# klae01/ddim-audio

Measured on AMD Instinct MI355X. Metric: DDIM denoising steps/sec (U-Net fwd/s), 1000-step sample, spectrogram batch, higher is better.
Workload: dtype bf16; 1 GPU; BASELINE configs[1]: batch 8/GPU x [2,1024,256] spectrograms, audio.yml U-Net (47.2M params, hash-filled weights; FNet GEMM operands bf16), generalized_steps eta=0 over the 1000-step schedule, one hipGraph per step (inside the forward two batch shards on two streams, fork mask 0x1003f); global_batch=8, t_size=1024, parallelism=batch-sharded x1, no collective in the loop

## Files before the change

ddim_audio_amd/_lib.py:

```python
import ctypes
import os
import re
from ctypes import Structure, c_char_p, c_double, c_float, c_int, c_longlong, c_uint, c_ulonglong, c_void_p

_HERE = os.path.dirname(os.path.abspath(__file__))
LIB_PATH = os.environ.get("DDIMX_LIB", os.path.join(_HERE, "libddimx.so"))
_HEADER = os.path.join(os.path.dirname(_HERE), "include", "ddimx.h")
_DISTILL_HEADER = os.path.join(os.path.dirname(_HERE), "include", "ddimx_distill.h")
_THRESHOLD_HEADER = os.path.join(os.path.dirname(_HERE), "include", "ddimx_threshold.h")
_SDE_HEADER = os.path.join(os.path.dirname(_HERE), "include", "ddimx_sde.h")
_BROWNIAN_HEADER = os.path.join(os.path.dirname(_HERE), "include", "ddimx_brownian.h")
_WINDOW_HEADER = os.path.join(os.path.dirname(_HERE), "include", "ddimx_window.h")
_WINDOW_INPAINT_HEADER = os.path.join(os.path.dirname(_HERE), "include", "ddimx_window_inpaint.h")
_UNIC_HEADER = os.path.join(os.path.dirname(_HERE), "include", "ddimx_unic.h")

_SCALARS = {"int": c_int, "unsigned": c_uint, "long long": c_longlong, "unsigned long long": c_ulonglong, "float": c_float,
            "double": c_double}
_RETURNS = {"int": c_int, "long long": c_longlong, "const char*": c_char_p}


def parse_header(text):
    def bad(what, decl):
        return RuntimeError(f"ddimx.h: {what}: `{decl}`")

    def split(decl):
        m = re.fullmatch(r"(.*?)\b(\w+)(?:\[(\w+)\])?", decl)
        if not m or not m.group(1):
            raise bad("cannot parse", decl)
        ctype, dim = m.group(1).strip(), m.group(3)
# ... 51 lines not shown
SDE_EXPORTS = tuple(_SDE_FUNCS)
with open(_BROWNIAN_HEADER) as _f:
    _BROWNIAN_CONSTS, _, _BROWNIAN_FUNCS = parse_header(_f.read())
globals().update(_BROWNIAN_CONSTS)
BROWNIAN_EXPORTS = tuple(_BROWNIAN_FUNCS)
with open(_WINDOW_HEADER) as _f:
    _, _, _WINDOW_FUNCS = parse_header(_f.read())
WINDOW_EXPORTS = tuple(_WINDOW_FUNCS)
with open(_WINDOW_INPAINT_HEADER) as _f:
    _, _, _WINDOW_INPAINT_FUNCS = parse_header(_f.read())
WINDOW_INPAINT_EXPORTS = tuple(_WINDOW_INPAINT_FUNCS)
with open(_UNIC_HEADER) as _f:
    _UNIC_CONSTS, _, _UNIC_FUNCS = parse_header(_f.read())
globals().update(_UNIC_CONSTS)
UNIC_EXPORTS = tuple(_UNIC_FUNCS)


class DdimxConfig(Structure):
    _fields_ = _STRUCTS["ddimx_config"]


class DdimxTables(Structure):
    _fields_ = _STRUCTS["ddimx_tables"]

    def __init__(self, posenc=None, dft_hidden=None, dft_seq=None, temb_table=None):
        super().__init__(posenc, dft_hidden, dft_seq, temb_table)


_lib = None


def load():
    global _lib
    if _lib is None:
        if not os.path.exists(LIB_PATH):
            raise RuntimeError(
                f"{LIB_PATH} not found: build it with `python -m ddim_audio_amd.build` "
                "(hipcc, gfx950). The HIP library is the only compute path of ddim_audio_amd.")
        lib = ctypes.CDLL(LIB_PATH)
        for name, (res, args) in (list(_FUNCS.items()) + list(_DISTILL_FUNCS.items()) + list(_THRESHOLD_FUNCS.items()) + list(_SDE_FUNCS.items())
                                  + list(_BROWNIAN_FUNCS.items()) + list(_WINDOW_FUNCS.items()) + list(_WINDOW_INPAINT_FUNCS.items())
                                  + list(_UNIC_FUNCS.items())):
            fn = getattr(lib, name)
            fn.restype, fn.argtypes = res, args
        if lib.ddimx_abi_version() != _CONSTS["DDIMX_ABI_VERSION"]:
            raise RuntimeError("libddimx ABI version mismatch")
        _lib = lib
    return _lib


def check(rc):
    if rc != 0:
        raise RuntimeError("libddimx: " + load().ddimx_last_error().decode(errors="replace"))


def ptr(t):
    return None if t is None else c_void_p(t.data_ptr())
# ... 6 lines not shown
```

ddim_audio_amd/build.py:

```python
import os
import subprocess
import sys
from concurrent.futures import ThreadPoolExecutor

HERE = os.path.dirname(os.path.abspath(__file__))
CSRC = os.path.join(HERE, "csrc")
OUT = os.path.join(HERE, "libddimx.so")
SOURCES = ["plan.cpp", "conv_dispatch.cpp", "blocks.cpp", "walk_infer.cpp", "walk_train.cpp", "ops.cpp", "samplers.cpp", "distill.cpp", "threshold.cpp", "sde.cpp", "brownian.cpp", "window_solver.cpp", "window_inpaint.cpp", "unic.cpp",
           "edge_conv.hip", "gn_kernels.hip", "fnet_pointwise.hip", "temb_kernels.hip", "step_kernels.hip", "tail_kernels.hip",
           "pack_kernels.hip", "wgrad_reduce.hip", "gemm.hip", "fnet_dense.hip", "conv_inst_bf16_c3.hip", "conv_inst_bf16_du.hip",
           "conv_inst_f32_c3.hip", "conv_inst_f32_du.hip", "conv_inst_bf16_c3b.hip", "conv_inst_bf16_wreg.hip", "conv_inst_bf16_pipe.hip", "conv_inst_f32_c3b.hip", "wgrad_inst_bf16.hip", "wgrad_inst_f32.hip",
           "inpaint_kernels.hip", "solver_kernels.hip", "noise_kernels.hip", "window_kernels.hip", "invert_kernels.hip", "pool_kernels.hip",
           "vpred_kernels.hip", "distill_kernels.hip", "threshold_kernels.hip", "sde_kernels.hip", "brownian_kernels.hip", "window_solver_kernels.hip", "window_inpaint_kernels.hip", "unic_kernels.hip"]
FLAGS = ["--offload-arch=gfx950", "-O3", "-std=c++17", "-fPIC", "-x", "hip", "-Wno-unused-result"]
EXTRA_FLAGS = {"conv_inst_bf16_pipe.hip": ["-fno-slp-vectorize", "-mllvm", "-amdgpu-mfma-vgpr-form=1"]}


def _stale(target, deps):
    if not os.path.exists(target):
        return True
    t = os.path.getmtime(target)
    return any(os.path.getmtime(d) > t for d in deps)


def build(force=False, verbose=True, jobs=None, stamp=False):
    global OUT, FLAGS
    hipcc = os.environ.get("HIPCC", "/opt/rocm/bin/hipcc")
    bdir = os.path.join(CSRC, "build_stamp" if stamp else "build")
    if stamp:
        OUT = os.path.join(HERE, "libddimx_stamp.so")
        FLAGS = FLAGS + ["-DDDIMX_STAMP"]
    os.makedirs(bdir, exist_ok=True)
    headers = [os.path.join(CSRC, f) for f in os.listdir(CSRC) if f.endswith(".h")]
    headers += [os.path.join(os.path.dirname(HERE), "include", h) for h in ("ddimx.h", "ddimx_distill.h", "ddimx_threshold.h", "ddimx_sde.h", "ddimx_brownian.h", "ddimx_window.h", "ddimx_window_inpaint.h", "ddimx_unic.h")]
    todo, objs = [], []
    for src in SOURCES:
        sp = os.path.join(CSRC, src)
        ob = os.path.join(bdir, src.rsplit(".", 1)[0] + ".o")
        objs.append(ob)
        if force or _stale(ob, [sp] + headers):
            todo.append((sp, ob))

    def cc(job):
        sp, ob = job
        cmd = [hipcc] + FLAGS + EXTRA_FLAGS.get(os.path.basename(sp), []) + ["-c", sp, "-o", ob]
        r = subprocess.run(cmd, capture_output=True, text=True)
        if r.returncode != 0:
            raise RuntimeError("hipcc failed for %s:\n%s" % (sp, r.stderr[-4000:]))
        return sp
# ... 19 lines not shown
```

ddim_audio_amd/csrc/edge_conv.h:

```cpp
#pragma once
#include "common.h"

namespace ddimx {

enum { EDGE_CONV_IN = 0, EDGE_CONV_OUT = 1, EDGE_CONV_OUT_BWD_DATA = 2, EDGE_CONV_IN_BWD_DATA = 3, EDGE_WGRAD = 4 };
struct EdgePlan {
    int variant;
    unsigned grid_x, grid_y;
    int threads, lds;
    int trips;
    int tiles_x, tiles_y;
    int partial_blocks;
    int reduce_blocks, reduce_unrolled, reduce_tail;
};
const char* edge_plan(int op, int dtype, int B, int C0, int Cio, int H, int W, int groups, EdgePlan* p);

hipError_t conv_in_launch(int dtype, const float* x, const float* w , const float* bias, void* out,
                          float* stats, int B, int cin, int C0, int H, int W, hipStream_t s, int groups = 0);
int conv_in_nparts(int H, int W);
hipError_t conv_out_launch(int dtype, const void* a, const void* b, const float* w ,
                           const float* bias, float* out, int B, int C0, int cout, int H, int W, hipStream_t s);

hipError_t conv_out_bwd_data_launch(int dtype, const float* d_eps, const float* w , void* ds, int B, int C0,
                                    int cout, int H, int W, hipStream_t s);
hipError_t conv_in_bwd_data_launch(int dtype, const void* dy, const float* w, float* dx, int B, int C0, int NI, int H, int W,
                                   hipStream_t s);
size_t edge_wgrad_partial_floats(int dtype, int B, int C, int NI, int H, int W);
hipError_t edge_wgrad_launch(int dtype, int mode, const void* g1, const void* g2, const float* S, float* partial, float* dW,
                             float* db, int B, int C, int NI, int H, int W, hipStream_t s);

}
```

ddim_audio_amd/csrc/edge_conv.hip:

```cpp
#include "edge_conv.h"
#include "gn_fused.h"
#include <stdarg.h>
#include <stdio.h>
#include <string.h>

namespace ddimx {

constexpr int kInPixPerBlock = 1024;
constexpr int kTileH = 8, kTileW = 32;
constexpr int kEdgeT = 16;
constexpr int kEdgeChunk = 32;
constexpr int kStripRows = 128;
static inline int edge_pixb(int dtype) { return dtype == DT_BF16 ? 64 : 32; }
int conv_in_nparts(int H, int W) { return (int)(((long long)H * W + kInPixPerBlock - 1) / kInPixPerBlock); }

template <typename T>
__global__ void __launch_bounds__(256) conv_in_kernel(const float* __restrict__ x, const float* __restrict__ w,
                                                      const float* __restrict__ bias, T* __restrict__ out,
                                                      float* __restrict__ stats, int cin, int C0, int H, int W,
                                                      int groups) {
    constexpr int EPB = Piece<T>::N;
    extern __shared__ __attribute__((aligned(16))) float lds[];
    float* wl = lds;
    float* red = lds + cin * 9 * C0;
// ... 216 lines not shown
        for (int k = 0; k < 9; ++k) {
            const float v = tile[((py + k / 3) * IW + px + k % 3) * LS + ci];
#pragma unroll
            for (int o = 0; o < 4; ++o)
                if (o < cout) acc[o] = fmaf(v, w[((size_t)k * cout + o) * C0 + ci], acc[o]);
        }
    }
    const int gy = y0 + py, gx = x0 + px;
    if (gy < H && gx < W) {
#pragma unroll
        for (int o = 0; o < 4; ++o)
            if (o < cout) out[(((size_t)b * cout + o) * H + gy) * W + gx] = acc[o];
    }
}

template <typename T, int C0, int NO, bool TWO, bool BIAS>
__device__ __forceinline__ void edge_tile_conv(const T* __restrict__ a, const T* __restrict__ b2, const float* __restrict__ w,
                                               const float* __restrict__ bias, float* __restrict__ out, int H, int W, int tiles_x,
                                               int tiles_y) {
    constexpr int EPB = Piece<T>::N, ES = sizeof(T);
    constexpr int IH = kTileH + 2, IW = kTileW + 2;
    constexpr int CPP = C0 / EPB, PS = C0 * ES + 16;
    __shared__ __attribute__((aligned(16))) char tile[IH * IW * PS];
    const int tid = threadIdx.x;
    const int tx = blockIdx.x % tiles_x, ty = (blockIdx.x / tiles_x) % tiles_y, b = blockIdx.x / (tiles_x * tiles_y);
    const int y0 = ty * kTileH, x0 = tx * kTileW;
    constexpr int NPIECE = IH * IW * CPP, NIT = (NPIECE + 255) / 256;
    uint4 va[NIT], vb[TWO ? NIT : 1];
    bool inb[NIT];
#pragma unroll
    for (int u = 0; u < NIT; ++u) {
        const int i0 = tid + u * 256, i = i0 < NPIECE ? i0 : NPIECE - 1;
        const int c = i % CPP, pix = i / CPP;
        const int gy = y0 - 1 + pix / IW, gx = x0 - 1 + pix % IW;
// ... 9 lines not shown
        uint4 v;
        if constexpr (TWO) {
            float f[EPB], k[EPB];
            Piece<T>::unpack(va[u], f);
            Piece<T>::unpack(vb[u], k);
#pragma unroll
            for (int j = 0; j < EPB; ++j) f[j] += k[j];
            v = Piece<T>::pack(f);
            if (!inb[u]) v = make_uint4(0, 0, 0, 0);
        } else {
            v = inb[u] ? va[u] : make_uint4(0, 0, 0, 0);
        }
        if (i < NPIECE) *(uint4*)(tile + (i / CPP) * PS + (i % CPP) * 16) = v;
    }
    __syncthreads();
    const int py = tid / kTileW, px = tid % kTileW;
    float acc[NO];
#pragma unroll
    for (int o = 0; o < NO; ++o) acc[o] = BIAS ? bias[o] : 0.f;
#pragma unroll 1
    for (int k = 0; k < 9; ++k) {
        const char* tp = tile + ((py + k / 3) * IW + px + k % 3) * PS;
        const float* wk = w + k * NO * C0;
#pragma unroll
        for (int c = 0; c < CPP; ++c) {
            float f[EPB];
            Piece<T>::unpack(*(const uint4*)(tp + c * 16), f);
#pragma unroll
            for (int j = 0; j < EPB; ++j)
#pragma unroll
                for (int o = 0; o < NO; ++o) acc[o] = fmaf(f[j], wk[o * C0 + c * EPB + j], acc[o]);
        }
    }
    const int gy = y0 + py, gx = x0 + px;
    if (gy < H && gx < W) {
#pragma unroll
        for (int o = 0; o < NO; ++o) out[(((size_t)b * NO + o) * H + gy) * W + gx] = acc[o];
    }
}

template <typename T, int C0, int COUT>
__global__ void __launch_bounds__(256) conv_out_fast_kernel(const T* __restrict__ a, const T* __restrict__ b2,
                                                            const float* __restrict__ w, const float* __restrict__ bias,
                                                            float* __restrict__ out, int H, int W, int tiles_x,
                                                            int tiles_y) {
    edge_tile_conv<T, C0, COUT, true, true>(a, b2, w, bias, out, H, W, tiles_x, tiles_y);
}

hipError_t conv_out_launch(int dtype, const void* a, const void* b, const float* w, const float* bias, float* out, int B,
                           int C0, int cout, int H, int W, hipStream_t s) {
    EdgePlan p;
    if (edge_plan(EDGE_CONV_OUT, dtype, B, C0, cout, H, W, 0, &p)) return hipErrorInvalidValue;
    const dim3 grid(p.grid_x);
    const int tiles_x = p.tiles_x, tiles_y = p.tiles_y;
    dispatch_dtype(dtype, [&](auto t) {
        using T = typename decltype(t)::type;
        if (p.variant)
            hipLaunchKernelGGL((conv_out_fast_kernel<T, 32, 2>), grid, dim3(256), 0, s, (const T*)a, (const T*)b, w, bias, out, H, W,
                               tiles_x, tiles_y);
        else
            hipLaunchKernelGGL(conv_out_kernel<T>, grid, dim3(256), p.lds, s, (const T*)a, (const T*)b, w, bias, out, C0, cout, H, W,
                               tiles_x, tiles_y);
    });
    return hipGetLastError();
}

template <typename T>
__global__ void __launch_bounds__(256) conv_out_bwd_data_kernel(const float* __restrict__ de, const float* __restrict__ w,
                                                                T* __restrict__ ds, int C0, int cout, int H, int W) {
    constexpr int EPB = Piece<T>::N;
    extern __shared__ float wl[];
    for (int i = threadIdx.x; i < 9 * cout * C0; i += 256) wl[i] = w[i];
    __syncthreads();
    const int CPP = C0 / EPB;
    const long long pieces = (long long)H * W * CPP;
    const int b = blockIdx.y;
    for (long long pc = blockIdx.x * 256ll + threadIdx.x; pc < pieces; pc += gridDim.x * 256ll) {
// ... 472 lines not shown
```

ddim_audio_amd/csrc/step_kernels.h:

```cpp
#pragma once
#include "common.h"

namespace ddimx {

hipError_t step_begin_launch(const float* coef, const int* step, int64_t* t, int B, int stride, hipStream_t s);
hipError_t step_end_launch(int* step, hipStream_t s);
hipError_t ddim_update_launch(float* xt, const float* et, const float* noise, float* x0, const float* coef,
                              const int* step, long long n, hipStream_t s);
hipError_t ddpm_update_launch(const float* x, const float* e, const float* noise, float* x0, float* xn, const float* coef,
                              const int* step, long long n, hipStream_t s);

}
```

ddim_audio_amd/csrc/step_kernels.hip:

```cpp
#include "step_kernels.h"
#include "step_math.h"

namespace ddimx {

__global__ void step_begin_kernel(const float* __restrict__ coef, const int* __restrict__ step, int64_t* __restrict__ t,
                                  int B, int stride) {
    const int i = blockIdx.x * blockDim.x + threadIdx.x;
    if (i < B) t[i] = (int64_t)coef[(size_t)step[0] * stride];
}
__global__ void step_end_kernel(int* step) { step[0] += 1; }

hipError_t step_begin_launch(const float* coef, const int* step, int64_t* t, int B, int stride, hipStream_t s) {
    hipLaunchKernelGGL(step_begin_kernel, dim3((B + 63) / 64), dim3(64), 0, s, coef, step, t, B, stride);
    return hipGetLastError();
}
hipError_t step_end_launch(int* step, hipStream_t s) {
    hipLaunchKernelGGL(step_end_kernel, dim3(1), dim3(1), 0, s, step);
    return hipGetLastError();
}

__global__ void __launch_bounds__(256) ddim_update_kernel(float* __restrict__ xt, const float* __restrict__ et,
                                                          const float* __restrict__ noise, float* __restrict__ x0,
                                                          const float* __restrict__ coef, const int* __restrict__ step,
                                                          long long n4) {
    const StepRow r = load_row(coef + (size_t)step[0] * 6, false);
    const bool add_z = noise != nullptr;
    for (long long i = (long long)blockIdx.x * 256 + threadIdx.x; i < n4; i += (long long)gridDim.x * 256) {
        float z[4] = {0.f, 0.f, 0.f, 0.f};
        if (add_z) load4(noise, (size_t)i, z);
        update4(xt, et, x0, nullptr, (size_t)i, r, false, false, false, add_z, z);
    }
}
// ... 36 lines not shown
```

ddim_audio_amd/csrc/walk_infer.cpp:

```cpp
#include "host.h"

void carve(const ddimx_ctx* c, char* base, int B, int T, Ws* w) {
    const ddimx_config& f = c->cfg;
    const int L = c->L;
    const size_t es = esz(c->dtype);
    Carver cv{base, 0};
    w->temb_h1 = (float*)cv.take((size_t)B * 512 * 4);
    w->temb_h2 = (float*)cv.take((size_t)B * 512 * 4);
    w->temb = (float*)cv.take((size_t)B * c->E * 4);
    const size_t lvl0 = (size_t)B * T * f.f_size * f.ch[0] * es;
    w->A = cv.take(lvl0);
    w->xd.resize(L); w->xu.resize(L);
    size_t stats_f = (size_t)B * conv_in_nparts(T, f.f_size) * (f.ch[0] * 2 > kGnSlab ? f.ch[0] * 2 : kGnSlab);
    size_t hmax = 0;
    int cmax = 0;
    for (int l = 0; l < L; ++l) {
        const int H = T >> l, W = f.f_size >> l, C = f.ch[l];
        const size_t bytes = (size_t)B * H * W * C * es;
        w->xd[l] = cv.take(bytes);
        w->xu[l] = cv.take(bytes);
        if (bytes > hmax) hmax = bytes;
        if (C > cmax) cmax = C;
        size_t s = conv_stats_floats(c->dtype, CONV3, C, C, B, H, W);
        if (s > stats_f) stats_f = s;
// ... 33 lines not shown
    {
        const int bf = c->fnet_bf16;
        const int shp[6][5] = {{(int)M, hid, c->width, 1, bf}, {2 * hid, S, hid, B, 0}, {S, hid, S, B, 0},
                               {(int)M, inter, hid, 1, bf}, {(int)M, hid, inter, 1, bf}, {(int)M, c->width, hid, 1, bf}};
        size_t mx = 0;
        for (auto& q : shp) {
            const size_t n = (size_t)kMaxSplitK * q[3] * q[0] * q[1];
            if (n > mx) mx = n;
        }
        w->gpart_per_sample = mx / B;
        w->gpart = (float*)cv.take(mx * 4);
    }
    w->total = cv.off;
}

extern "C" {

long long ddimx_workspace_bytes(ddimx_handle h, int B, int T) {
    if (!h || B < 1 || T < 1) return 0;
    Ws w;
    carve(h, nullptr, B, T, &w);
    return (long long)w.total;
}

int ddimx_unet_fwd(ddimx_handle h, const void* packed, const ddimx_tables* tables, void* workspace,
                   long long workspace_bytes, const float* x, const int64_t* t, float* eps, int B, int T, void* stream) {
    return ddimx_unet_fwd_forked(h, packed, tables, workspace, workspace_bytes, x, t, eps, B, T, stream, nullptr, nullptr, 0, 0);
}

int ddimx_unet_fwd_forked(ddimx_handle h, const void* packed, const ddimx_tables* tables, void* workspace, long long workspace_bytes,
                          const float* x, const int64_t* t, float* eps, int B, int T, void* stream, void* aux_stream,
                          void* const* events, int n_events, unsigned fork_mask) {
    if (!h || !packed || !tables || !workspace || !x || !t || !eps) return fail("ddimx_unet_fwd: null argument");
    const ddimx_ctx* c = h;
    const ddimx_config& f = c->cfg;
    const int L = c->L;
    CHK(check_shape(c, B, T));
    Ws w;
    CHK(carve_checked("ddimx_unet_fwd", carve, c, workspace, workspace_bytes, B, T, &w));
    hipStream_t s = (hipStream_t)stream, sa = (hipStream_t)aux_stream;
    if (!sa || !events || n_events < 2 || B < 2) fork_mask = 0;
    fork_mask &= 0xFFFFFu;
    int ev_used = 0;
    const int dt = c->dtype;
    const size_t es = esz(dt);
    const int bh = B / 2;
    bool forked = false;
    auto sync_for = [&](bool sharded) -> int {
// ... 14 lines not shown
    auto act_bytes = [&](int l) { return (size_t)(T >> l) * (f.f_size >> l) * f.ch[l] * es; };
    struct Lane { int b0, n; hipStream_t st; };
    auto for_lanes = [&](bool sharded, auto&& op) -> int {
        CHK(sync_for(sharded));
        if (!sharded) return op(Lane{0, B, s});
        CHK(op(Lane{bh, B - bh, sa}));
        CHK(op(Lane{0, bh, s}));
        return 0;
    };
    auto at = [&](const void* p, size_t per_sample, int b0) { return (void*)((char*)const_cast<void*>(p) + per_sample * b0); };
    int cur = 0;
    auto stats_of = [&](const Lane& ln, int which) { return (which ? w.stats2 : w.stats) + w.stats_per_sample * ln.b0; };
    auto scale_of = [&](const Lane& ln) { return w.scale + (size_t)w.cmax * ln.b0; };
    auto shift_of = [&](const Lane& ln) { return w.shift + (size_t)w.cmax * ln.b0; };

    if (tables->temb_table) {
        HIPCHK(temb_gather_launch(tables->temb_table, t, w.temb, B, c->E, s));
    } else {
        CHK(run_temb(pf(c, packed, c->te), t, pf(c, packed, c->tw[0]), pf(c, packed, c->tb[0]), pf(c, packed, c->tw[1]),
                     pf(c, packed, c->tb[1]), pf(c, packed, c->tw[2]), pf(c, packed, c->tb[2]), w.temb_h1, w.temb_h2, w.temb,
                     B, 128, 512, c->E, s));
    }
    auto resblock = [&](int l, const void* in, void* out, const float* temb_chunk, const RBW& rbw, int np, int cs, bool want_stats,
                        int* ynp) -> int {
        const int H = T >> l, W = f.f_size >> l, C = f.ch[l];
        return for_lanes(lvl_on(l), [&](const Lane& ln) -> int {
            return run_resblock(dt, C, at(in, act_bytes(l), ln.b0), at(out, act_bytes(l), ln.b0), temb_chunk + (size_t)c->E * ln.b0, c->E,
                                rb_ptrs(c, packed, rbw), at(w.h1, w.h_per_sample, ln.b0), at(w.h2, w.h_per_sample, ln.b0), stats_of(ln, cur),
                                scale_of(ln), shift_of(ln), np, cs, want_stats, ynp, ln.n, H, W, ln.st, nullptr, stats_of(ln, cur ^ 1));
        });
    };
// ... 64 lines not shown
            np = ynp; cs = C;
        }
        if (l > 0) {
            CHK(for_lanes(lvl_on(l - 1), [&](const Lane& ln) -> int {
                ConvCall u = up4_call(dt, C, f.ch[l - 1], at(w.xu[l], act_bytes(l), ln.b0), pv(c, packed, c->up_w[l]),
                                      at(w.xd[l - 1], act_bytes(l - 1), ln.b0), at(w.xu[l - 1], act_bytes(l - 1), ln.b0), ln.n, H, W);
                u.bias = pf(c, packed, c->up_b[l]);
                u.stats = stats_of(ln, 0);
                u.groups = true;
                u.wf = frag_of(c, packed, c->up_w[l]);
                return run_conv(u, ln.st, &np, &cs);
            }));
            cur = 0;
        }
    }
    CHK(for_lanes(lvl_on(0), [&](const Lane& ln) -> int {
        HIPCHK(conv_out_launch(dt, at(w.xu[0], act_bytes(0), ln.b0), at(w.A, act_bytes(0), ln.b0), pf(c, packed, c->out_w),
                               pf(c, packed, c->out_b), eps + in_per * ln.b0, ln.n, f.ch[0], f.in_channels, T, f.f_size, ln.st));
        return 0;
    }));
    CHK(sync_for(false));
    return 0;
}

int ddimx_fnet_fwd(ddimx_handle h, const void* packed, const ddimx_tables* tables, void* workspace, long long workspace_bytes,
                   const void* x, float* out, int B, int T, void* stream) {
    if (!h || !packed || !tables || !workspace || !x || !out) return fail("ddimx_fnet_fwd: null argument");
    const ddimx_ctx* c = h;
    const int L = c->L;
    CHK(check_shape(c, B, T));
    Ws w;
    CHK(carve_checked("ddimx_fnet_fwd", carve, c, workspace, workspace_bytes, B, T, &w));
    hipStream_t s = (hipStream_t)stream;
    const int S = T >> (L - 1);
    CHK(run_fnet(c, packed, tables, w, x, B, S, s));
    HIPCHK(hipMemcpyAsync(out, w.O, (size_t)B * S * c->width * 4, hipMemcpyDeviceToDevice, s));
    return 0;
}
// ... 3 lines not shown
```

ddim_audio_amd/model.py:

```python
import math
from collections import OrderedDict

import torch
import torch.nn as nn
from torch.autograd.function import once_differentiable

_POS_CH = 128
_EMB_CH = 512
_GROUPS = 8


def embedding_sizes(mcfg):
    e = [c for r, c in zip(mcfg.res, mcfg.ch) for _ in range(r)]
    return e + e[::-1]


def _rb(inv, p, c, k):
    for i in range(3):
        inv[f"{p}norm.{i}.weight"] = (c,)
        if i < 2:
            inv[f"{p}norm.{i}.bias"] = (c,)
    inv[f"{p}conv.0.weight"] = (c, c, k, k)
    inv[f"{p}conv.1.weight"] = (c, c, k, k)
    inv[f"{p}conv.1.bias"] = (c,)
# ... 537 lines not shown
            nlev = len(self.config.ch)
            s = t_len >> (nlev - 1)
            fr = self.config.f_size >> (nlev - 1)
            c_last = self.config.ch[-1]
            hid = self.config.transformers.kwargs.hidden_size
            pe = _posenc_table(s, c_last * fr, c_last, fr).to(device)
            ch, sh = _dft_tables(hid)
            cs, ss = _dft_tables(s)
            import numpy as np
            dh = torch.from_numpy(np.stack([ch, sh], axis=1).reshape(2 * hid, hid)).to(device)
            ds = torch.from_numpy(np.concatenate([cs, -ss], axis=1)).contiguous().to(device)
            self._tables = {key: (pe, dh, ds)}
            self._gen += 1
        return self._tables[key]

    def forward_slot(self, input, t, slot, out=None):
        return self.forward(input, t, _slot=slot, _fork=False, _out=out)

    def forward(self, input, t, _slot=0, _fork=True, _ctx=None, _out=None):
        from . import _lib
        if not input.is_cuda:
            raise RuntimeError("ddim_audio_amd.Model computes only through libddimx on a ROCm GPU; got a CPU tensor "
                               "(there is no CPU fallback)")
        if input.dtype != torch.float32:
            raise RuntimeError("the network boundary is fp32 [B,C,T,F] (activations inside use config.model.dtype)")
        b, c, t_len, f = input.shape
        if c != self.config.channels or f != self.config.f_size:
            raise RuntimeError(f"expected [B,{self.config.channels},T,{self.config.f_size}], got {tuple(input.shape)}")
        lib = self._ensure_handle()
        dev = input.device
        with torch.cuda.device(dev):
            self._ensure_packed(lib, dev)
            pe, dh, ds = self._ensure_tables(t_len, dev)
            wsp = self.reserve(dev, b, t_len, _slot)
            x = input.contiguous()
            tt = t.to(device=dev, dtype=torch.int64).contiguous()
            if self.training and torch.is_grad_enabled():
                self._ensure_packed_bwd(lib, dev)
                params = [p for _, p in self.named_parameters()]
                if getattr(self, "_alias_leaves", False):
                    params = self._leaf_aliases = [p.detach().requires_grad_(True) for p in params]
                return _UNetTrainFn.apply(self, x, tt, (pe, dh, ds), True, *params)
            if torch.is_grad_enabled() and input.requires_grad:
                self._ensure_packed_bwd(lib, dev)
                return _UNetTrainFn.apply(self, x, tt, (pe, dh, ds), False, *[p for _, p in self.named_parameters()])
            if _out is not None:
                if _out.shape != x.shape or _out.dtype != torch.float32 or not _out.is_contiguous() or _out.device != dev:
                    raise RuntimeError("_out must be a contiguous fp32 tensor of the input's shape on its device")
                out = _out
            else:
                out = torch.empty_like(x)
            tt_ptr = self._temb_table.data_ptr() if (not self.training and getattr(self, "_temb_table", None) is not None) else None
            tables = _lib.DdimxTables(pe.data_ptr(), dh.data_ptr(), ds.data_ptr(), tt_ptr)
            import ctypes
            mask = self.fork_mask if (_fork and b >= 4) else 0
            fc = None
            if mask:
                fc = _ctx if torch.cuda.is_current_stream_capturing() else self._eager_context(dev)
            if fc is not None:
                _lib.check(lib.ddimx_unet_fwd_forked(self._handle, _lib.ptr(self._packed), ctypes.byref(tables), _lib.ptr(wsp),
                                                     wsp.numel(), _lib.ptr(x), _lib.ptr(tt), _lib.ptr(out), b, t_len, _lib.stream(),
                                                     ctypes.c_void_p(fc.aux_handle), fc.event_array(), len(fc.events), mask))
            else:
                _lib.check(lib.ddimx_unet_fwd(self._handle, _lib.ptr(self._packed), ctypes.byref(tables),
                                              _lib.ptr(wsp), wsp.numel(), _lib.ptr(x), _lib.ptr(tt),
                                              _lib.ptr(out), b, t_len, _lib.stream()))
        return out
```

ddim_audio_amd/sampler.py:

```python
import os

import numpy as np
import torch

from . import _lib
from .graphs import GraphOwner
from .schedule import X0Threshold, check_prediction, check_threshold, ddim_coefficients, ddpm_coefficients, threshold_rank, v_table


def _selected(select_index, index, n):
    return select_index is None or index in select_index or index - n in select_index


def _device(model, x):
    if isinstance(model, torch.nn.Module):
        p = next(model.parameters(), None)
        if p is not None and p.is_cuda:
            return p.device
    return x.device if x.is_cuda else torch.device("cuda", torch.cuda.current_device())


def _check_noise(noise, noise_fn):
    if noise is None:
        return
# ... 62 lines not shown
        for index in range(n_iter):
            for _ in range(per):
                stepper.step()
            if _selected(select_index, index, n_iter):
                x0_preds.append(stepper.x0.to("cpu"))
                xs.append(stepper.xt.to("cpu"))
        if finish is not None:
            finish(stepper)
    finally:
        stepper.close()
    return xs, x0_preds


class DDIMStepper(GraphOwner):

    def __init__(self, model, xt, coef64, use_graph=True, noise_fn=None, slot=0, fork=True, noise=None, net_in=None, v_table=None, threshold=None):
        super().__init__(model)
        _check_noise(noise, noise_fn)
        self.lib = _lib.load()
        self.xt = xt
        self.net_in = net_in = xt if net_in is None else net_in
        dev = xt.device
        self.coef = torch.from_numpy(np.ascontiguousarray(coef64, dtype=np.float32)).to(dev).contiguous()
        self.n_iter = self.coef.size(0)
        self.counter = torch.zeros(1, dtype=torch.int32, device=dev)
        self.t = torch.zeros(net_in.size(0), dtype=torch.int64, device=dev)
        self.x0 = torch.empty_like(xt)
        self.noise_fn = noise_fn
        self.use_graph = (use_graph and noise_fn is None and os.environ.get("DDIMX_GRAPH", "1") != "0"
                          and not torch.cuda.is_current_stream_capturing())
        self.done = 0
        self._capture_pending = self.use_graph
        self.native = hasattr(model, "forward_slot")
        self.slot, self.fork = slot, fork
        self.vtab = None
        if v_table is not None:
            vt = np.ascontiguousarray(v_table, dtype=np.float32)
            if vt.ndim != 2 or vt.shape[0] < 1 or vt.shape[1] != 2:
                raise ValueError("v_table must be [n_table, 2] rows (s1, s2) (schedule.v_table)")
            self.vtab = torch.from_numpy(vt).to(dev).contiguous()
# ... 66 lines not shown
        _lib.check(self.lib.ddimxq_threshold_eps(_lib.ptr(x), _lib.ptr(out), _lib.ptr(eps), _lib.ptr(self.scale), *tab, *shape))
        return eps

    def _update(self, et, noise, st):
        xt = self.xt
        _lib.check(self.lib.ddimx_ddim_update(_lib.ptr(xt), _lib.ptr(et), _lib.ptr(noise), _lib.ptr(self.x0), _lib.ptr(self.coef),
                                              _lib.ptr(self.counter), xt.numel(), st))

    def _begin(self, st):
        t = self.t
        _lib.check(self.lib.ddimx_step_begin_ex(_lib.ptr(self.coef), self.coef.size(1), _lib.ptr(self.counter), _lib.ptr(t), t.numel(), st))

    def _end(self, st):
        _lib.check(self.lib.ddimx_step_end(_lib.ptr(self.counter), st))

    def _launch(self, noise):
        st = _lib.stream()
        self._begin(st)
        self._gather(st)
        et = self._to_eps(self._forward(), st)
        self._update(et, self._draw(noise), st)
        self._end(st)

    def _captured_refs(self):
        return self.model.captured_refs() if self.native else None

    def rewind(self):
        self.counter.zero_()

    def _stale(self):
        if not self.native:
# ... 87 lines not shown
```

Baseline: 2343 sample-fwd/s.

## Fuse DDIM step begin/update into U-Net temb gather and output conv

Adds a step-frame path in which the U-Net forward folds the DDIM step into its own kernels. The timestep read from the coefficient table is fused with the temb gather, and the DDIM x/x0 update is fused into the output convolution epilogue. The separate step_begin, eps write/read and ddim_update kernels are removed from each captured step graph. When the ticket option is on, the counter advance is done by the last workgroup through an atomic ticket. With the default ticket off, a separate step_end launch remains, and there are extra register and load costs in the conv_out kernel.

```diff
diff --git a/ddim_audio_amd/_lib.py b/ddim_audio_amd/_lib.py
--- a/ddim_audio_amd/_lib.py
+++ b/ddim_audio_amd/_lib.py
@@ -13,6 +13,7 @@
 _WINDOW_HEADER = os.path.join(os.path.dirname(_HERE), "include", "ddimx_window.h")
 _WINDOW_INPAINT_HEADER = os.path.join(os.path.dirname(_HERE), "include", "ddimx_window_inpaint.h")
 _UNIC_HEADER = os.path.join(os.path.dirname(_HERE), "include", "ddimx_unic.h")
+_STEP_HEADER = os.path.join(os.path.dirname(_HERE), "include", "ddimx_step.h")
 
 _SCALARS = {"int": c_int, "unsigned": c_uint, "long long": c_longlong, "unsigned long long": c_ulonglong, "float": c_float,
             "double": c_double}
@@ -94,6 +95,9 @@
     _UNIC_CONSTS, _, _UNIC_FUNCS = parse_header(_f.read())
 globals().update(_UNIC_CONSTS)
 UNIC_EXPORTS = tuple(_UNIC_FUNCS)
+with open(_STEP_HEADER) as _f:
+    _, _STEP_STRUCTS, _STEP_FUNCS = parse_header(_f.read())
+STEP_EXPORTS = tuple(_STEP_FUNCS)
 
 
 class DdimxConfig(Structure):
@@ -105,6 +109,10 @@
 
     def __init__(self, posenc=None, dft_hidden=None, dft_seq=None, temb_table=None):
         super().__init__(posenc, dft_hidden, dft_seq, temb_table)
+
+
+class DdimxfFrame(Structure):
+    _fields_ = _STEP_STRUCTS["ddimxf_frame"]
 
 
 _lib = None
@@ -120,7 +128,7 @@
         lib = ctypes.CDLL(LIB_PATH)
         for name, (res, args) in (list(_FUNCS.items()) + list(_DISTILL_FUNCS.items()) + list(_THRESHOLD_FUNCS.items()) + list(_SDE_FUNCS.items())
                                   + list(_BROWNIAN_FUNCS.items()) + list(_WINDOW_FUNCS.items()) + list(_WINDOW_INPAINT_FUNCS.items())
-                                  + list(_UNIC_FUNCS.items())):
+                                  + list(_UNIC_FUNCS.items()) + list(_STEP_FUNCS.items())):
             fn = getattr(lib, name)
             fn.restype, fn.argtypes = res, args
         if lib.ddimx_abi_version() != _CONSTS["DDIMX_ABI_VERSION"]:
diff --git a/ddim_audio_amd/build.py b/ddim_audio_amd/build.py
--- a/ddim_audio_amd/build.py
+++ b/ddim_audio_amd/build.py
@@ -6,7 +6,7 @@
 HERE = os.path.dirname(os.path.abspath(__file__))
 CSRC = os.path.join(HERE, "csrc")
 OUT = os.path.join(HERE, "libddimx.so")
-SOURCES = ["plan.cpp", "conv_dispatch.cpp", "blocks.cpp", "walk_infer.cpp", "walk_train.cpp", "ops.cpp", "samplers.cpp", "distill.cpp", "threshold.cpp", "sde.cpp", "brownian.cpp", "window_solver.cpp", "window_inpaint.cpp", "unic.cpp",
+SOURCES = ["plan.cpp", "conv_dispatch.cpp", "blocks.cpp", "walk_infer.cpp", "walk_train.cpp", "ops.cpp", "samplers.cpp", "distill.cpp", "threshold.cpp", "sde.cpp", "brownian.cpp", "window_solver.cpp", "window_inpaint.cpp", "unic.cpp", "step_frame.cpp",
            "edge_conv.hip", "gn_kernels.hip", "fnet_pointwise.hip", "temb_kernels.hip", "step_kernels.hip", "tail_kernels.hip",
            "pack_kernels.hip", "wgrad_reduce.hip", "gemm.hip", "fnet_dense.hip", "conv_inst_bf16_c3.hip", "conv_inst_bf16_du.hip",
            "conv_inst_f32_c3.hip", "conv_inst_f32_du.hip", "conv_inst_bf16_c3b.hip", "conv_inst_bf16_wreg.hip", "conv_inst_bf16_pipe.hip", "conv_inst_f32_c3b.hip", "wgrad_inst_bf16.hip", "wgrad_inst_f32.hip",
@@ -32,7 +32,7 @@
         FLAGS = FLAGS + ["-DDDIMX_STAMP"]
     os.makedirs(bdir, exist_ok=True)
     headers = [os.path.join(CSRC, f) for f in os.listdir(CSRC) if f.endswith(".h")]
-    headers += [os.path.join(os.path.dirname(HERE), "include", h) for h in ("ddimx.h", "ddimx_distill.h", "ddimx_threshold.h", "ddimx_sde.h", "ddimx_brownian.h", "ddimx_window.h", "ddimx_window_inpaint.h", "ddimx_unic.h")]
+    headers += [os.path.join(os.path.dirname(HERE), "include", h) for h in ("ddimx.h", "ddimx_distill.h", "ddimx_threshold.h", "ddimx_sde.h", "ddimx_brownian.h", "ddimx_window.h", "ddimx_window_inpaint.h", "ddimx_unic.h", "ddimx_step.h")]
     todo, objs = [], []
     for src in SOURCES:
         sp = os.path.join(CSRC, src)
diff --git a/ddim_audio_amd/csrc/edge_conv.h b/ddim_audio_amd/csrc/edge_conv.h
--- a/ddim_audio_amd/csrc/edge_conv.h
+++ b/ddim_audio_amd/csrc/edge_conv.h
@@ -20,6 +20,10 @@
 int conv_in_nparts(int H, int W);
 hipError_t conv_out_launch(int dtype, const void* a, const void* b, const float* w ,
                            const float* bias, float* out, int B, int C0, int cout, int H, int W, hipStream_t s);
+hipError_t conv_out_ddim_launch(int dtype, const void* a, const void* b, const float* w, const float* bias, float* eps, float* xt,
+                                const float* noise, float* x0, const float* coef, int stride, int* step, int* ticket, long long total,
+                                int B, int C0, int cout, int H, int W, hipStream_t s);
+long long conv_out_tiles(int H, int W);
 
 hipError_t conv_out_bwd_data_launch(int dtype, const float* d_eps, const float* w , void* ds, int B, int C0,
                                     int cout, int H, int W, hipStream_t s);
diff --git a/ddim_audio_amd/csrc/edge_conv.hip b/ddim_audio_amd/csrc/edge_conv.hip
--- a/ddim_audio_amd/csrc/edge_conv.hip
+++ b/ddim_audio_amd/csrc/edge_conv.hip
@@ -1,5 +1,6 @@
 #include "edge_conv.h"
 #include "gn_fused.h"
+#include "step_math.h"
 #include <stdarg.h>
 #include <stdio.h>
 #include <string.h>
@@ -254,10 +255,15 @@
     }
 }
 
-template <typename T, int C0, int NO, bool TWO, bool BIAS>
-__device__ __forceinline__ void edge_tile_conv(const T* __restrict__ a, const T* __restrict__ b2, const float* __restrict__ w,
-                                               const float* __restrict__ bias, float* __restrict__ out, int H, int W, int tiles_x,
-                                               int tiles_y) {
+struct EdgePixel { int b, gy, gx; };
+__device__ __forceinline__ EdgePixel edge_tile_pixel(int tiles_x, int tiles_y) {
+    const int tx = blockIdx.x % tiles_x, ty = (blockIdx.x / tiles_x) % tiles_y, b = blockIdx.x / (tiles_x * tiles_y);
+    return {b, ty * kTileH + (int)threadIdx.x / kTileW, tx * kTileW + (int)threadIdx.x % kTileW};
+}
+template <typename T, int C0, int NO, bool TWO, bool BIAS, typename Staged>
+__device__ __forceinline__ void edge_tile_acc(const T* __restrict__ a, const T* __restrict__ b2, const float* __restrict__ w,
+                                              const float* __restrict__ bias, int H, int W, int tiles_x, int tiles_y, float (&acc)[NO],
+                                              Staged&& staged) {
     constexpr int EPB = Piece<T>::N, ES = sizeof(T);
     constexpr int IH = kTileH + 2, IW = kTileW + 2;
     constexpr int CPP = C0 / EPB, PS = C0 * ES + 16;
@@ -297,8 +303,8 @@
         if (i < NPIECE) *(uint4*)(tile + (i / CPP) * PS + (i % CPP) * 16) = v;
     }
     __syncthreads();
+    staged();
     const int py = tid / kTileW, px = tid % kTileW;
-    float acc[NO];
 #pragma unroll
     for (int o = 0; o < NO; ++o) acc[o] = BIAS ? bias[o] : 0.f;
 #pragma unroll 1
@@ -315,10 +321,17 @@
                 for (int o = 0; o < NO; ++o) acc[o] = fmaf(f[j], wk[o * C0 + c * EPB + j], acc[o]);
         }
     }
-    const int gy = y0 + py, gx = x0 + px;
-    if (gy < H && gx < W) {
-#pragma unroll
-        for (int o = 0; o < NO; ++o) out[(((size_t)b * NO + o) * H + gy) * W + gx] = acc[o];
+}
+template <typename T, int C0, int NO, bool TWO, bool BIAS>
+__device__ __forceinline__ void edge_tile_conv(const T* __restrict__ a, const T* __restrict__ b2, const float* __restrict__ w,
+                                               const float* __restrict__ bias, float* __restrict__ out, int H, int W, int tiles_x,
+                                               int tiles_y) {
+    float acc[NO];
+    edge_tile_acc<T, C0, NO, TWO, BIAS>(a, b2, w, bias, H, W, tiles_x, tiles_y, acc, [] {});
+    const EdgePixel p = edge_tile_pixel(tiles_x, tiles_y);
+    if (p.gy < H && p.gx < W) {
+#pragma unroll
+        for (int o = 0; o < NO; ++o) out[(((size_t)p.b * NO + o) * H + p.gy) * W + p.gx] = acc[o];
     }
 }
 
@@ -328,6 +341,47 @@
                                                             float* __restrict__ out, int H, int W, int tiles_x,
                                                             int tiles_y) {
     edge_tile_conv<T, C0, COUT, true, true>(a, b2, w, bias, out, H, W, tiles_x, tiles_y);
+}
+
+template <typename T, int C0, int COUT>
+__global__ void __launch_bounds__(256, 6) conv_out_ddim_kernel(const T* __restrict__ a, const T* __restrict__ b2,
+                                                            const float* __restrict__ w, const float* __restrict__ bias, float* eps,
+                                                            float* xt, const float* __restrict__ noise, float* __restrict__ x0p,
+                                                            const float* __restrict__ coef, int stride, int* step, int* ticket,
+                                                            int total, int H, int W, int tiles_x, int tiles_y) {
+    static_assert(COUT == 2, "the two channels of a pixel ride in two of update4_core's four slots");
+    const int row = step[0];
+    const StepRow r = load_row(coef + (size_t)row * stride, false);
+    const bool add_z = noise != nullptr;
+    const size_t plane = (size_t)H * W;
+    size_t at = 0;
+    bool inside = false;
+    float xa = 0.f, xb = 0.f, za = 0.f, zb = 0.f;
+    float acc[COUT];
+    edge_tile_acc<T, C0, COUT, true, true>(a, b2, w, bias, H, W, tiles_x, tiles_y, acc, [&]() __attribute__((always_inline)) {
+        const EdgePixel p = edge_tile_pixel(tiles_x, tiles_y);
+        inside = p.gy < H && p.gx < W;
+        at = ((size_t)p.b * COUT * H + (p.gy < H ? p.gy : H - 1)) * W + (p.gx < W ? p.gx : W - 1);
+        xa = xt[at];
+        xb = xt[at + plane];
+        if (add_z) { za = noise[at]; zb = noise[at + plane]; }
+    });
+    float x[4] = {xa, xb, 0.f, 0.f}, z[4] = {za, zb, 0.f, 0.f}, e[4] = {acc[0], acc[1], 0.f, 0.f}, m0[4];
+    update4_core(x, e, z, z, m0, r, false, false, add_z, z);
+    if (inside) {
+#pragma unroll
+        for (int o = 0; o < COUT; ++o) {
+            if (eps) eps[at + o * plane] = acc[o];
+            x0p[at + o * plane] = m0[o];
+            xt[at + o * plane] = x[o];
+        }
+    }
+    asm volatile("" ::"s"(row) : "memory");
+    __syncthreads();
+    if (ticket && threadIdx.x == 0 && __hip_atomic_fetch_add(ticket, 1, __ATOMIC_RELAXED, __HIP_MEMORY_SCOPE_AGENT) == total - 1) {
+        __hip_atomic_store(ticket, 0, __ATOMIC_RELAXED, __HIP_MEMORY_SCOPE_AGENT);
+        step[0] = row + 1;
+    }
 }
 
 hipError_t conv_out_launch(int dtype, const void* a, const void* b, const float* w, const float* bias, float* out, int B,
@@ -344,6 +398,27 @@
         else
             hipLaunchKernelGGL(conv_out_kernel<T>, grid, dim3(256), p.lds, s, (const T*)a, (const T*)b, w, bias, out, C0, cout, H, W,
                                tiles_x, tiles_y);
+    });
+    return hipGetLastError();
+}
+
+long long conv_out_tiles(int H, int W) {
+    EdgePlan p;
+    if (edge_plan(EDGE_CONV_OUT, DT_F32, 1, 32, 2, H, W, 0, &p)) return -1;
+    return (long long)p.tiles_x * p.tiles_y;
+}
+hipError_t conv_out_ddim_launch(int dtype, const void* a, const void* b, const float* w, const float* bias, float* eps, float* xt,
+                                const float* noise, float* x0, const float* coef, int stride, int* step, int* ticket, long long total,
+                                int B, int C0, int cout, int H, int W, hipStream_t s) {
+    EdgePlan p;
+    if (edge_plan(EDGE_CONV_OUT, dtype, B, C0, cout, H, W, 0, &p) || !p.variant) return hipErrorInvalidValue;
+    if (stride < 6 || (ticket && (total < (long long)p.grid_x || total > 0x7fffffffll))) return hipErrorInvalidValue;
+    const dim3 grid(p.grid_x);
+    const int tiles_x = p.tiles_x, tiles_y = p.tiles_y;
+    dispatch_dtype(dtype, [&](auto t) {
+        using T = typename decltype(t)::type;
+        hipLaunchKernelGGL((conv_out_ddim_kernel<T, 32, 2>), grid, dim3(256), 0, s, (const T*)a, (const T*)b, w, bias, eps, xt, noise, x0,
+                           coef, stride, step, ticket, (int)total, H, W, tiles_x, tiles_y);
     });
     return hipGetLastError();
 }
diff --git a/ddim_audio_amd/csrc/step_frame.cpp b/ddim_audio_amd/csrc/step_frame.cpp
--- /dev/null
+++ b/ddim_audio_amd/csrc/step_frame.cpp
@@ -0,0 +1,33 @@
+#include "host.h"
+#include "../../include/ddimx_step.h"
+
+extern "C" {
+
+int ddimxf_step_begin_temb(const float* coef, int row_stride, const int* counter, int64_t* t, const float* table, float* temb, int b0,
+                           int n, int E, void* stream) {
+    if (!coef || !counter || !t || !table || !temb) return fail("ddimxf_step_begin_temb: null argument");
+    if (row_stride < 1) return fail("ddimxf_step_begin_temb: row_stride = %d must be positive", row_stride);
+    if (b0 < 0 || n < 1 || n > 65535) return fail("ddimxf_step_begin_temb: samples [%d, %d + %d): b0 >= 0, 1 <= n <= 65535", b0, b0, n);
+    if (E < 4 || E % 4) return fail("ddimxf_step_begin_temb: E = %d must be a positive multiple of 4", E);
+    HIPCHK(step_begin_temb_launch(coef, row_stride, counter, t + b0, table, temb + (size_t)E * b0, n, E, (hipStream_t)stream));
+    return 0;
+}
+
+long long ddimxf_conv_out_tiles(int H, int W) { return H < 1 || W < 1 ? -1 : conv_out_tiles(H, W); }
+
+int ddimxf_conv_out_ddim(int dtype, const void* a, const void* b, const float* w_packed, const float* bias, float* eps, float* xt,
+                         const float* noise, float* x0, const float* coef, int row_stride, int* counter, int* ticket,
+                         long long ticket_total, int B, int C0, int Cout, int H, int W, void* stream) {
+    if (!a || !b || !w_packed || !bias || !xt || !x0 || !coef || !counter) return fail("ddimxf_conv_out_ddim: null argument");
+    EdgePlan p;
+    if (const char* why = edge_plan(EDGE_CONV_OUT, dtype, B, C0, Cout, H, W, 0, &p)) return fail("ddimxf_conv_out_ddim: %s", why);
+    if (!p.variant) return fail("ddimxf_conv_out_ddim: C0 = %d, Cout = %d: only (32, 2) has the fused kernel", C0, Cout);
+    if (row_stride < 6) return fail("ddimxf_conv_out_ddim: row_stride = %d, a DDIM row has 6 values", row_stride);
+    if (ticket && (ticket_total < (long long)p.grid_x || ticket_total > 0x7fffffffll))
+        return fail("ddimxf_conv_out_ddim: ticket_total = %lld, this launch alone has %u workgroups", ticket_total, p.grid_x);
+    HIPCHK(conv_out_ddim_launch(dtype, a, b, w_packed, bias, eps, xt, noise, x0, coef, row_stride, counter, ticket, ticket_total, B, C0,
+                                Cout, H, W, (hipStream_t)stream));
+    return 0;
+}
+
+}
diff --git a/ddim_audio_amd/csrc/step_kernels.h b/ddim_audio_amd/csrc/step_kernels.h
--- a/ddim_audio_amd/csrc/step_kernels.h
+++ b/ddim_audio_amd/csrc/step_kernels.h
@@ -5,6 +5,8 @@
 
 hipError_t step_begin_launch(const float* coef, const int* step, int64_t* t, int B, int stride, hipStream_t s);
 hipError_t step_end_launch(int* step, hipStream_t s);
+hipError_t step_begin_temb_launch(const float* coef, int stride, const int* step, int64_t* t, const float* table, float* temb, int n,
+                                  int E, hipStream_t s);
 hipError_t ddim_update_launch(float* xt, const float* et, const float* noise, float* x0, const float* coef,
                               const int* step, long long n, hipStream_t s);
 hipError_t ddpm_update_launch(const float* x, const float* e, const float* noise, float* x0, float* xn, const float* coef,
diff --git a/ddim_audio_amd/csrc/step_kernels.hip b/ddim_audio_amd/csrc/step_kernels.hip
--- a/ddim_audio_amd/csrc/step_kernels.hip
+++ b/ddim_audio_amd/csrc/step_kernels.hip
@@ -16,6 +16,23 @@
 }
 hipError_t step_end_launch(int* step, hipStream_t s) {
     hipLaunchKernelGGL(step_end_kernel, dim3(1), dim3(1), 0, s, step);
+    return hipGetLastError();
+}
+
+__global__ void __launch_bounds__(256) step_begin_temb_kernel(const float* __restrict__ coef, const int* __restrict__ step, int stride,
+                                                              int64_t* __restrict__ t, const float* __restrict__ table,
+                                                              float* __restrict__ temb, int E) {
+    const int b = blockIdx.y;
+    const int64_t tv = (int64_t)coef[(size_t)step[0] * stride];
+    if (blockIdx.x == 0 && threadIdx.x == 0) t[b] = tv;
+    const float4* src = (const float4*)(table + (size_t)tv * E);
+    float4* dst = (float4*)(temb + (size_t)b * E);
+    for (int i = blockIdx.x * 256 + threadIdx.x; i < E / 4; i += gridDim.x * 256) dst[i] = src[i];
+}
+hipError_t step_begin_temb_launch(const float* coef, int stride, const int* step, int64_t* t, const float* table, float* temb, int n,
+                                  int E, hipStream_t s) {
+    if (E % 4 || n < 1 || n > 65535) return hipErrorInvalidValue;
+    hipLaunchKernelGGL(step_begin_temb_kernel, dim3((E / 4 + 255) / 256, n), dim3(256), 0, s, coef, step, stride, t, table, temb, E);
     return hipGetLastError();
 }
 
diff --git a/ddim_audio_amd/csrc/walk_infer.cpp b/ddim_audio_amd/csrc/walk_infer.cpp
--- a/ddim_audio_amd/csrc/walk_infer.cpp
+++ b/ddim_audio_amd/csrc/walk_infer.cpp
@@ -1,4 +1,5 @@
 #include "host.h"
+#include "../../include/ddimx_step.h"
 
 void carve(const ddimx_ctx* c, char* base, int B, int T, Ws* w) {
     const ddimx_config& f = c->cfg;
@@ -71,6 +72,10 @@
     w->total = cv.off;
 }
 
+static int unet_walk(ddimx_handle h, const void* packed, const ddimx_tables* tables, void* workspace, long long workspace_bytes,
+                     const float* x, const int64_t* t, float* eps, const ddimxf_frame* fr, int B, int T, void* stream,
+                     void* aux_stream, void* const* events, int n_events, unsigned fork_mask);
+
 extern "C" {
 
 long long ddimx_workspace_bytes(ddimx_handle h, int B, int T) {
@@ -89,6 +94,31 @@
                           const float* x, const int64_t* t, float* eps, int B, int T, void* stream, void* aux_stream,
                           void* const* events, int n_events, unsigned fork_mask) {
     if (!h || !packed || !tables || !workspace || !x || !t || !eps) return fail("ddimx_unet_fwd: null argument");
+    return unet_walk(h, packed, tables, workspace, workspace_bytes, x, t, eps, nullptr, B, T, stream, aux_stream, events, n_events,
+                     fork_mask);
+}
+
+static bool frame_ok(const ddimx_ctx* c) { return c->cfg.ch[0] == 32 && c->cfg.in_channels == 2; }
+int ddimxf_frame_ok(ddimx_handle h) { return h && frame_ok(h) ? 1 : 0; }
+
+int ddimxf_unet_fwd_step(ddimx_handle h, const void* packed, const void* tables, void* workspace, long long workspace_bytes,
+                         const ddimxf_frame* fr, int B, int T, void* stream, void* aux_stream, void* const* events, int n_events,
+                         unsigned fork_mask) {
+    if (!h || !packed || !tables || !workspace || !fr) return fail("ddimxf_unet_fwd_step: null argument");
+    if (!fr->coef || !fr->counter || !fr->t || !fr->xt || !fr->x0) return fail("ddimxf_unet_fwd_step: null in the frame");
+    if (fr->row_stride < 6) return fail("ddimxf_unet_fwd_step: row_stride = %d, a DDIM row has 6 values", fr->row_stride);
+    if (!((const ddimx_tables*)tables)->temb_table) return fail("ddimxf_unet_fwd_step: the frame needs tables->temb_table (eval mode)");
+    if (!frame_ok(h))
+        return fail("ddimxf_unet_fwd_step: ch[0] = %d, in_channels = %d have no fused output conv (32, 2)", h->cfg.ch[0], h->cfg.in_channels);
+    return unet_walk(h, packed, (const ddimx_tables*)tables, workspace, workspace_bytes, fr->xt, fr->t, fr->eps, fr, B, T, stream,
+                     aux_stream, events, n_events, fork_mask);
+}
+
+}
+
+static int unet_walk(ddimx_handle h, const void* packed, const ddimx_tables* tables, void* workspace, long long workspace_bytes,
+                     const float* x, const int64_t* t, float* eps, const ddimxf_frame* fr, int B, int T, void* stream,
+                     void* aux_stream, void* const* events, int n_events, unsigned fork_mask) {
     const ddimx_ctx* c = h;
     const ddimx_config& f = c->cfg;
     const int L = c->L;
@@ -133,7 +163,13 @@
     auto scale_of = [&](const Lane& ln) { return w.scale + (size_t)w.cmax * ln.b0; };
     auto shift_of = [&](const Lane& ln) { return w.shift + (size_t)w.cmax * ln.b0; };
 
-    if (tables->temb_table) {
+    if (fr) {
+        CHK(for_lanes(lvl_on(0), [&](const Lane& ln) -> int {
+            HIPCHK(step_begin_temb_launch(fr->coef, fr->row_stride, fr->counter, fr->t + ln.b0, tables->temb_table,
+                                          w.temb + (size_t)c->E * ln.b0, ln.n, c->E, ln.st));
+            return 0;
+        }));
+    } else if (tables->temb_table) {
         HIPCHK(temb_gather_launch(tables->temb_table, t, w.temb, B, c->E, s));
     } else {
         CHK(run_temb(pf(c, packed, c->te), t, pf(c, packed, c->tw[0]), pf(c, packed, c->tb[0]), pf(c, packed, c->tw[1]),
@@ -228,14 +264,25 @@
             cur = 0;
         }
     }
+    const long long tickets = fr ? conv_out_tiles(T, f.f_size) * B : 0;
     CHK(for_lanes(lvl_on(0), [&](const Lane& ln) -> int {
-        HIPCHK(conv_out_launch(dt, at(w.xu[0], act_bytes(0), ln.b0), at(w.A, act_bytes(0), ln.b0), pf(c, packed, c->out_w),
-                               pf(c, packed, c->out_b), eps + in_per * ln.b0, ln.n, f.ch[0], f.in_channels, T, f.f_size, ln.st));
+        const void *xu = at(w.xu[0], act_bytes(0), ln.b0), *xa = at(w.A, act_bytes(0), ln.b0);
+        const size_t o = in_per * ln.b0;
+        if (fr)
+            HIPCHK(conv_out_ddim_launch(dt, xu, xa, pf(c, packed, c->out_w), pf(c, packed, c->out_b), eps ? eps + o : nullptr, fr->xt + o,
+                                        fr->noise ? fr->noise + o : nullptr, fr->x0 + o, fr->coef, fr->row_stride, fr->counter,
+                                        fr->ticket, tickets, ln.n, f.ch[0], f.in_channels, T, f.f_size, ln.st));
+        else
+            HIPCHK(conv_out_launch(dt, xu, xa, pf(c, packed, c->out_w), pf(c, packed, c->out_b), eps + o, ln.n, f.ch[0], f.in_channels, T,
+                                   f.f_size, ln.st));
         return 0;
     }));
     CHK(sync_for(false));
+    if (fr && !fr->ticket) HIPCHK(step_end_launch(fr->counter, s));
     return 0;
 }
+
+extern "C" {
 
 int ddimx_fnet_fwd(ddimx_handle h, const void* packed, const ddimx_tables* tables, void* workspace, long long workspace_bytes,
                    const void* x, float* out, int B, int T, void* stream) {
diff --git a/ddim_audio_amd/model.py b/ddim_audio_amd/model.py
--- a/ddim_audio_amd/model.py
+++ b/ddim_audio_amd/model.py
@@ -575,10 +575,14 @@
             self._gen += 1
         return self._tables[key]
 
+    def step_frame_ok(self):
+        return (not self.training and getattr(self, "_temb_table", None) is not None
+                and bool(self._ensure_handle().ddimxf_frame_ok(self._handle)))
+
     def forward_slot(self, input, t, slot, out=None):
         return self.forward(input, t, _slot=slot, _fork=False, _out=out)
 
-    def forward(self, input, t, _slot=0, _fork=True, _ctx=None, _out=None):
+    def forward(self, input, t, _slot=0, _fork=True, _ctx=None, _out=None, _frame=None):
         from . import _lib
         if not input.is_cuda:
             raise RuntimeError("ddim_audio_amd.Model computes only through libddimx on a ROCm GPU; got a CPU tensor "
@@ -588,6 +592,8 @@
         b, c, t_len, f = input.shape
         if c != self.config.channels or f != self.config.f_size:
             raise RuntimeError(f"expected [B,{self.config.channels},T,{self.config.f_size}], got {tuple(input.shape)}")
+        if _frame is not None and (self.training or input.requires_grad or not input.is_contiguous()):
+            raise RuntimeError("_frame is an inference step in place on a contiguous input: eval mode, no gradient")
         lib = self._ensure_handle()
         dev = input.device
         with torch.cuda.device(dev):
@@ -609,7 +615,7 @@
                 if _out.shape != x.shape or _out.dtype != torch.float32 or not _out.is_contiguous() or _out.device != dev:
                     raise RuntimeError("_out must be a contiguous fp32 tensor of the input's shape on its device")
                 out = _out
-            else:
+            elif _frame is None:
                 out = torch.empty_like(x)
             tt_ptr = self._temb_table.data_ptr() if (not self.training and getattr(self, "_temb_table", None) is not None) else None
             tables = _lib.DdimxTables(pe.data_ptr(), dh.data_ptr(), ds.data_ptr(), tt_ptr)
@@ -618,6 +624,11 @@
             fc = None
             if mask:
                 fc = _ctx if torch.cuda.is_current_stream_capturing() else self._eager_context(dev)
+            if _frame is not None:
+                aux = (ctypes.c_void_p(fc.aux_handle), fc.event_array(), len(fc.events), mask) if fc is not None else (None, None, 0, 0)
+                _lib.check(lib.ddimxf_unet_fwd_step(self._handle, _lib.ptr(self._packed), ctypes.byref(tables), _lib.ptr(wsp), wsp.numel(),
+                                                    ctypes.byref(_frame), b, t_len, _lib.stream(), *aux))
+                return None
             if fc is not None:
                 _lib.check(lib.ddimx_unet_fwd_forked(self._handle, _lib.ptr(self._packed), ctypes.byref(tables), _lib.ptr(wsp),
                                                      wsp.numel(), _lib.ptr(x), _lib.ptr(tt), _lib.ptr(out), b, t_len, _lib.stream(),
diff --git a/ddim_audio_amd/sampler.py b/ddim_audio_amd/sampler.py
--- a/ddim_audio_amd/sampler.py
+++ b/ddim_audio_amd/sampler.py
@@ -100,6 +100,8 @@
 
 class DDIMStepper(GraphOwner):
 
+    frame_ticket = False
+
     def __init__(self, model, xt, coef64, use_graph=True, noise_fn=None, slot=0, fork=True, noise=None, net_in=None, v_table=None, threshold=None):
         super().__init__(model)
         _check_noise(noise, noise_fn)
@@ -110,6 +112,8 @@
         self.coef = torch.from_numpy(np.ascontiguousarray(coef64, dtype=np.float32)).to(dev).contiguous()
         self.n_iter = self.coef.size(0)
         self.counter = torch.zeros(1, dtype=torch.int32, device=dev)
+        self.ticket = torch.zeros(1, dtype=torch.int32, device=dev) if type(self) is DDIMStepper else None
+        self._frame = None
         self.t = torch.zeros(net_in.size(0), dtype=torch.int64, device=dev)
         self.x0 = torch.empty_like(xt)
         self.noise_fn = noise_fn
@@ -206,7 +210,22 @@
     def _end(self, st):
         _lib.check(self.lib.ddimx_step_end(_lib.ptr(self.counter), st))
 
+    def _step_frame(self):
+        if (type(self) is not DDIMStepper or not self.native or self.vtab is not None or self.threshold is not None
+                or self.net_in is not self.xt or not torch.cuda.is_current_stream_capturing() or not self.model.step_frame_ok()):
+            return None
+        if self._frame is None:
+            p = lambda t: None if t is None else t.data_ptr()
+            self._frame = _lib.DdimxfFrame(p(self.coef), p(self.counter), p(self.t), p(self.xt), p(self.x0), p(self.noise_buf), None,
+                                           p(self.ticket) if self.frame_ticket else None, self.coef.size(1))
+        return self._frame
+
     def _launch(self, noise):
+        frame = self._step_frame()
+        if frame is not None:
+            self._draw(noise)
+            self.model(self.xt, self.t, _slot=self.slot, _fork=self.fork, _ctx=self._ctx, _frame=frame)
+            return
         st = _lib.stream()
         self._begin(st)
         self._gather(st)
diff --git a/include/ddimx_step.h b/include/ddimx_step.h
--- /dev/null
+++ b/include/ddimx_step.h
@@ -0,0 +1,39 @@
+#ifndef DDIMX_STEP_H
+#define DDIMX_STEP_H
+
+#include <stdint.h>
+
+#ifdef __cplusplus
+extern "C" {
+#endif
+
+typedef struct {
+    const float* coef;
+    int* counter;
+    int64_t* t;
+    float* xt;
+    float* x0;
+    const float* noise;
+    float* eps;
+    int* ticket;
+    int row_stride;
+} ddimxf_frame;
+
+int ddimxf_step_begin_temb(const float* coef, int row_stride, const int* counter, int64_t* t, const float* table, float* temb, int b0,
+                           int n, int E, void* stream);
+
+int ddimxf_conv_out_ddim(int dtype, const void* a, const void* b, const float* w_packed, const float* bias, float* eps, float* xt,
+                         const float* noise, float* x0, const float* coef, int row_stride, int* counter, int* ticket,
+                         long long ticket_total, int B, int C0, int Cout, int H, int W, void* stream);
+long long ddimxf_conv_out_tiles(int H, int W);
+
+int ddimxf_frame_ok(struct ddimx_ctx* h);
+
+int ddimxf_unet_fwd_step(struct ddimx_ctx* h, const void* packed, const void* tables, void* workspace, long long workspace_bytes,
+                         const ddimxf_frame* frame, int B, int T, void* stream, void* aux_stream, void* const* events, int n_events,
+                         unsigned fork_mask);
+
+#ifdef __cplusplus
+}
+#endif
+#endif
```

New measurement: 2345 sample-fwd/s, median of 5. About the same (+0.1%).
